# whcorkran/mamba-TTS-project

Measured on AMD Instinct MI355X. Metric: audio tokens/sec (teacher-forced fwd+bwd) per GPU; decode_step p50 latency, higher is better.
Workload: dtype bf16; 1 GPU; C2: MambaTTSDecoder 12L d_model=1024 fwd+bwd+clip+Adam, B=8/GPU T_audio=2048 T_text=128; model=MambaTTSDecoder-12L-d1024, global_batch=8, seq_len=2048, parallelism=dp1

## Files before the change

### include/mtts.h

```cpp
#ifndef MTTS_H
#define MTTS_H

#include <stdint.h>

#ifdef __cplusplus
extern "C" {
#endif

#define MTTS_ABI_VERSION 15

enum { MTTS_F32 = 0, MTTS_BF16 = 1 };
enum {
  MTTS_OK = 0,
  MTTS_EINVAL = -22,
  MTTS_EUNSUPPORTED = -95,
  MTTS_ELAUNCH = -5
};

int mtts_abi_version(void);
const char* mtts_last_error(void);

enum {
  MTTS_OVR_AUTO = -1,
  MTTS_OVR_SCAN_PATH = 0,
// ... 255 lines not shown
int mtts_embed_table_grad(const int64_t* ids, int64_t n, const void* g, int dtype, int64_t g_rs, int d, int vocab,
                          float* out, void* workspace, void* stream);

typedef struct {
  int M, N, K, act;
  int64_t ldx, ldw, ldy;
  const void* x;
  const void* W;
  const void* bias;
  void* y;
  int conv_dim;
  float* conv_state;
  const float* conv_w;
  const float* conv_b;
  void* u;
  int64_t ldu;
  const float* ln_w;
  const float* ln_b;
  float ln_eps;
  const void* gamma;
  const void* beta;
  int64_t ld_gb;
  const void* res;
  int64_t ld_res;
  int kgroups;
  float* splitk_slab;
  int* splitk_count;
  int w_packed;
  int x_packed;
  void* y_packed;
  void* u_packed;
} MttsRowsArgs;

int mtts_gemm_rows(const MttsRowsArgs* a, void* stream);

typedef struct {
  int64_t rows;
  int vocab;
  int dtype;
  int64_t ld;
  const void* logits;
  const int64_t* targets;
  int ignore_index;
  float* loss;
  float* lse;
  float* workspace;
} MttsCrossEntropyArgs;

int64_t mtts_cross_entropy_workspace(int64_t rows);
int mtts_cross_entropy_fwd(const MttsCrossEntropyArgs* a, void* stream);
int mtts_cross_entropy_bwd(const MttsCrossEntropyArgs* a, const float* grad_loss, void* dlogits, int64_t ld_dlogits,
                           void* stream);

int64_t mtts_pack_rows_bytes(int N, int K);
int mtts_pack_rows_weight(const void* W, int64_t ldw, int N, int K, void* out, void* stream);


#define MTTS_GEMM_NT 0
#define MTTS_GEMM_TN 1
#define MTTS_GEMM_EPI_BIAS 1
#define MTTS_GEMM_EPI_GELU 2
#define MTTS_GEMM_EPI_DGELU 4
typedef struct {
  int m, n, k;
  int layout;
  int splits;
  int epilogue;
  int out_dtype;
  int bias_dtype;
  int64_t lda, ldb, ldc, ld_aux;
  const void* a;
  const void* b;
  void* c;
  const void* bias;
  void* aux;
  void* workspace;
  float beta;
} MttsGemmArgs;

int64_t mtts_gemm_workspace(const MttsGemmArgs* a);
int mtts_gemm(const MttsGemmArgs* a, void* stream);

int mtts_gemm_grouped(const MttsGemmArgs* probs, int n, void* stream);

#define MTTS_CONVGEMM_NN 2
#define MTTS_CONVGEMM_BIAS 1
#define MTTS_CONVGEMM_RELU 2
#define MTTS_CONVGEMM_DRELU 4
typedef struct {
  const void* ptr;
  int64_t seg_rows, seg_stride, row_stride;
  int32_t halo_c, halo_p;
} MttsRowMap;
typedef struct {
  int layout;
  int m, n, k;
  MttsRowMap a, b, c, aux;
  const float* bias;
  int epilogue;
  float beta;
  int splits;
  void* workspace;
  float* colsum_a;
} MttsConvGemmArgs;
int64_t mtts_convgemm_workspace(const MttsConvGemmArgs* a);
int mtts_convgemm(const MttsConvGemmArgs* a, void* stream);

#define MTTS_SKINNY_N 0
#define MTTS_SKINNY_SMALL_K 1
#define MTTS_SKINNY_TN 2
typedef struct {
  int mode;
  int m, n, k;
  int c_dtype;
  float beta;
  int64_t lda, ldb, ldc;
  const void* a;
  const void* b;
  void* c;
  void* workspace;
  int trans_c;
  int reserved_;
} MttsSkinnyArgs;

int64_t mtts_gemm_skinny_workspace(const MttsSkinnyArgs* a);
int mtts_gemm_skinny(const MttsSkinnyArgs* a, void* stream);

typedef struct {
  int64_t n;
  int dtype;
  float p;
  uint64_t seed;
  const void* x;
  void* y;
  const void* pre;
  int group;
  int x_rep;
  int x_inner;
  int reserved_;
  const int64_t* seed_in;
  int64_t* seed_out;
} MttsDropoutArgs;

int mtts_dropout(const MttsDropoutArgs* a, void* stream);

typedef struct {
  int rows, vocab;
  int dtype;
  int top_k;
  int64_t ld;
  const void* logits;
  const float* bias;
  int64_t bias_ld;
  float temperature;
  float top_p;
  const int64_t* seed;
  int* step;
  int advance;
  int step0;
  int* pos;
  int64_t* tokens;
  int64_t tok_stride;
  int64_t* history;
  int64_t hist_ld;
  int hist_cols;
  int eos_id;
// ... 14 lines not shown
```

### mamba-tts-project_amd/mtts/_lib.py

```python
from __future__ import annotations

import contextlib
import ctypes as C
import os

import torch

_HERE = os.path.dirname(os.path.abspath(__file__))
LIB_PATH = os.environ.get("MTTS_LIB", os.path.join(_HERE, "libmtts.so"))
ABI_VERSION = 15

F32, BF16 = 0, 1
i32, i64, f32, vp = C.c_int, C.c_int64, C.c_float, C.c_void_p


class ScanFwdArgs(C.Structure):
    _fields_ = [("batch", i32), ("dim", i32), ("seqlen", i32), ("dstate", i32),
                ("dtype_io", i32), ("dtype_bc", i32), ("delta_softplus", i32), ("ckpt_chunk", i32),
                ("a_is_log", i32), ("reserved_", i32), ("u_bs", i64), ("u_ls", i64), ("delta_bs", i64), ("delta_ls", i64),
                ("z_bs", i64), ("z_ls", i64), ("out_bs", i64), ("out_ls", i64),
                ("B_bs", i64), ("B_ls", i64), ("C_bs", i64), ("C_ls", i64),
                ("u", vp), ("delta", vp), ("A", vp), ("Bm", vp), ("Cm", vp), ("D", vp), ("z", vp),
                ("delta_bias", vp), ("h0", vp), ("out", vp), ("last_state", vp), ("ckpt", vp),
                ("workspace", vp), ("seqlens", vp)]
# ... 72 lines not shown
class RowMap(C.Structure):
    _fields_ = [("ptr", vp), ("seg_rows", i64), ("seg_stride", i64), ("row_stride", i64), ("halo_c", i32),
                ("halo_p", i32)]


class ConvGemmArgs(C.Structure):
    _fields_ = [("layout", i32), ("m", i32), ("n", i32), ("k", i32), ("a", RowMap), ("b", RowMap), ("c", RowMap),
                ("aux", RowMap), ("bias", vp), ("epilogue", i32), ("beta", f32), ("splits", i32),
                ("workspace", vp), ("colsum_a", vp)]


class SkinnyArgs(C.Structure):
    _fields_ = [("mode", i32), ("m", i32), ("n", i32), ("k", i32), ("c_dtype", i32), ("beta", f32),
                ("lda", i64), ("ldb", i64), ("ldc", i64), ("a", vp), ("b", vp), ("c", vp), ("workspace", vp),
                ("trans_c", i32), ("reserved_", i32)]


class LNArgs(C.Structure):
    _fields_ = [("rows", i32), ("cols", i32), ("dtype", i32), ("rows_per_group", i32), ("eps", f32),
                ("x_rs", i64), ("res_rs", i64), ("xsum_rs", i64), ("y_rs", i64), ("gb_rs", i64),
                ("x", vp), ("res", vp), ("x_sum", vp), ("w", vp), ("b", vp), ("gamma", vp), ("beta", vp),
                ("gb_dtype", i32), ("y", vp), ("mean", vp), ("rstd", vp)]


class LNBwdArgs(C.Structure):
    _fields_ = [("f", LNArgs), ("dy", vp), ("dy_rs", i64), ("dx_acc", vp), ("dxacc_rs", i64),
                ("dx", vp), ("dx_rs", i64), ("dw", vp), ("db", vp), ("dgamma", vp), ("dbeta", vp),
                ("workspace", vp), ("dx_colsum", vp), ("dgb_rs", i64)]


class AttnFwdArgs(C.Structure):
    _fields_ = [("batch", i32), ("heads", i32), ("head_dim", i32), ("q_len", i32), ("kv_len", i32),
                ("dtype", i32), ("scale", f32),
                ("q_bs", i64), ("q_ls", i64), ("k_bs", i64), ("k_ls", i64), ("v_bs", i64), ("v_ls", i64),
                ("o_bs", i64), ("o_ls", i64), ("mask_bs", i64),
                ("q", vp), ("k", vp), ("v", vp), ("key_padding_mask", vp), ("out", vp), ("lse", vp),
                ("out_packed", vp), ("kv_hs", i64)]


class AttnQProjArgs(C.Structure):
    _fields_ = [("f", AttnFwdArgs), ("x", vp), ("x_rs", i64), ("wq", vp), ("bq", vp), ("ln_w", vp), ("ln_b", vp),
                ("eps", f32), ("d_model", i32)]


class AttnBwdArgs(C.Structure):
    _fields_ = [("f", AttnFwdArgs), ("dout", vp), ("do_bs", i64), ("do_ls", i64),
                ("dq", vp), ("dq_bs", i64), ("dq_ls", i64), ("dk", vp), ("dk_bs", i64), ("dk_ls", i64),
                ("dv", vp), ("dv_bs", i64), ("dv_ls", i64), ("workspace", vp)]


class CastDesc(C.Structure):
    _fields_ = [("src", vp), ("dst", vp), ("dstT", vp), ("rows", i32), ("cols", i32), ("tile0", i64)]


class AdamTensor(C.Structure):
    _fields_ = [("p", vp), ("g", vp), ("m", vp), ("v", vp), ("n", i64), ("chunk0", i64)]


_SIGS = {
    "mtts_abi_version": ([], i32),
    "mtts_last_error": ([], C.c_char_p),
    "mtts_set_override": ([i32, i32], i32),
    "mtts_get_override": ([i32], i32),
    "mtts_selective_scan_fwd_workspace": ([i32, i32, i32, i32], i64),
    "mtts_selective_scan_fwd": ([C.POINTER(ScanFwdArgs), vp], i32),
    "mtts_selective_scan_bwd_workspace": ([i32, i32, i32, i32], i64),
    "mtts_selective_scan_bwd": ([C.POINTER(ScanBwdArgs), vp], i32),
    "mtts_causal_conv1d_fwd": ([C.POINTER(ConvFwdArgs), vp], i32),
    "mtts_causal_conv1d_bwd_workspace": ([i32, i32, i32, i32], i64),
    "mtts_causal_conv1d_bwd": ([C.POINTER(ConvBwdArgs), vp], i32),
    "mtts_causal_conv1d_update": ([C.POINTER(ConvUpdateArgs), vp], i32),
    "mtts_selective_state_update": ([C.POINTER(StateUpdateArgs), vp], i32),
    "mtts_layernorm_fwd": ([C.POINTER(LNArgs), vp], i32),
    "mtts_gemm_rows": ([C.POINTER(RowsArgs), vp], i32),
    "mtts_pack_rows_bytes": ([i32, i32], i64),
    "mtts_cross_entropy_workspace": ([i64], i64),
    "mtts_cross_entropy_fwd": ([C.POINTER(CrossEntropyArgs), vp], i32),
    "mtts_cross_entropy_bwd": ([C.POINTER(CrossEntropyArgs), vp, vp, i64, vp], i32),
    "mtts_layernorm_rows_packed": ([C.POINTER(LNArgs), vp, vp], i32),
    "mtts_pack_rows_weight": ([vp, i64, i32, i32, vp, vp], i32),
    "mtts_gemm_workspace": ([C.POINTER(GemmArgs)], i64),
    "mtts_gemm": ([C.POINTER(GemmArgs), vp], i32),
    "mtts_gemm_grouped": ([C.POINTER(GemmArgs), i32, vp], i32),
    "mtts_convgemm": ([C.POINTER(ConvGemmArgs), vp], i32),
    "mtts_convgemm_workspace": ([C.POINTER(ConvGemmArgs)], i64),
    "mtts_gemm_skinny": ([C.POINTER(SkinnyArgs), vp], i32),
    "mtts_gemm_skinny_workspace": ([C.POINTER(SkinnyArgs)], i64),
    "mtts_layernorm_bwd_workspace": ([i32, i32, i32], i64),
    "mtts_layernorm_bwd": ([C.POINTER(LNBwdArgs), vp], i32),
    "mtts_colsum_workspace": ([i32, i32, i32], i64),
    "mtts_colsum": ([vp, i32, i32, i32, i64, i32, vp, i64, vp, vp], i32),
    "mtts_attention_fwd": ([C.POINTER(AttnFwdArgs), vp], i32),
    "mtts_attention_decode_qproj": ([C.POINTER(AttnQProjArgs), vp], i32),
    "mtts_attention_bwd_workspace": ([i32, i32, i32, i32, i32, i32], i64),
    "mtts_attention_bwd": ([C.POINTER(AttnBwdArgs), vp], i32),
    "mtts_adam_chunks": ([i64], i64),
    "mtts_adam_workspace": ([i64], i64),
    "mtts_clip_adam": ([vp, i32, i64, vp, f32, f32, f32, f32, f32, f32, vp, vp, vp], i32),
    "mtts_embed_sum": ([vp, i64, vp, vp, vp, vp, vp, i32, i32, i32, i32, vp, i32, i64, vp, vp], i32),
    "mtts_embed_sum_at": ([vp, i64, vp, vp, vp, vp, vp, i32, i32, i32, i32, vp, i32, i64, vp, i64, i32, vp], i32),
    "mtts_embed_table_grad_workspace": ([i64, i32, i32], i64),
    "mtts_embed_table_grad": ([vp, i64, vp, i32, i64, i32, i32, vp, vp, vp], i32),
    "mtts_cast_tiles": ([i32, i32], i64),
    "mtts_cast_bf16_multi": ([vp, i32, i64, vp], i32),
    "mtts_length_regulate_lengths": ([vp, i64, i32, i32, vp, vp], i32),
    "mtts_length_regulate_fwd": ([vp, i32, i32, i32, i32, i64, i64, vp, i64, i32, vp, i64, i64, vp], i32),
    "mtts_length_regulate_bwd": ([vp, i32, i32, i32, i32, i64, i64, vp, i64, i32, vp, i64, i64, vp], i32),
    "mtts_dropout": ([C.POINTER(DropoutArgs), vp], i32),
    "mtts_sample_tokens": ([C.POINTER(SampleArgs), vp], i32),
}

_lib = None


def lib():
    global _lib
    if _lib is None:
        if not os.path.exists(LIB_PATH):
            raise RuntimeError(f"libmtts.so not found at {LIB_PATH}; run __graft_entry__.build() "
                               "(make -C mamba-tts-project_amd/mtts/csrc)")
        L = C.CDLL(LIB_PATH)
        if not hasattr(L, "mtts_embed_sum_at"):
            raise RuntimeError(f"{LIB_PATH} is stale: it was built before mtts_embed_sum_at (ragged prompts) was "
                               "added; rebuild it with __graft_entry__.build() "
                               "(make -C mamba-tts-project_amd/mtts/csrc)")
        for name, (argt, rest) in _SIGS.items():
            fn = getattr(L, name)
            fn.argtypes = argt
            fn.restype = rest
        v = L.mtts_abi_version()
        if v != ABI_VERSION:
            raise RuntimeError(f"libmtts ABI {v} != expected {ABI_VERSION}")
        _lib = L
    return _lib


def exported_symbols():
    return list(_SIGS)


def call(name, args):
    L = lib()
    stream = torch.cuda.current_stream().cuda_stream
    rc = getattr(L, name)(C.byref(args), C.c_void_p(stream))
    if rc != 0:
        raise RuntimeError(f"{name} failed ({rc}): {L.mtts_last_error().decode()}")


def call_raw(name, *args):
    L = lib()
    rc = getattr(L, name)(*args, C.c_void_p(torch.cuda.current_stream().cuda_stream))
    if rc != 0:
        raise RuntimeError(f"{name} failed ({rc}): {L.mtts_last_error().decode()}")


OVERRIDES = {"scan_path": 0, "scan_p": 1, "scan_segs": 2, "scan_bwd_segs": 3, "gemm_narrow": 4,
             "attn_chunks": 5, "attn_bwd": 6, "attn_generic": 7, "conv_untiled": 8, "gemm_tile": 9,
             "attn_dq_dma": 10}
SCAN_C1, SCAN_W2, SCAN_NARROW = 1, 2, 3
ATTN_BWD_FUSED, ATTN_BWD_SPLIT = 1, 2


@contextlib.contextmanager
def override(**paths):
    L = lib()
    old = {}
    try:
        for k, v in paths.items():
            old[k] = L.mtts_set_override(OVERRIDES[k], -1 if v is None else int(v))
        yield
    finally:
        for k, v in old.items():
            L.mtts_set_override(OVERRIDES[k], v)


def dtype_code(t: torch.Tensor) -> int:
    if t.dtype == torch.float32:
        return F32
    if t.dtype == torch.bfloat16:
        return BF16
    raise TypeError(f"unsupported dtype {t.dtype} (libmtts takes float32 / bfloat16)")


def ptr(t):
    return None if t is None else t.data_ptr()
```

### mamba-tts-project_amd/mtts/csrc/gemm.hip

```cpp
#include "common.h"

#include <type_traits>

namespace mtts {
namespace {

typedef short s16x8 __attribute__((ext_vector_type(8)));
typedef short s16x4 __attribute__((ext_vector_type(4)));
typedef __bf16 bf16x8 __attribute__((ext_vector_type(8)));
typedef float f32x4 __attribute__((ext_vector_type(4)));
typedef __attribute__((address_space(3))) s16x4 lds_s16x4;
typedef __attribute__((address_space(3))) s16x8 lds_s16x8;

constexpr int kThreads = 512;
constexpr int kTile = 256;
constexpr int kBK = 64;
constexpr int kRegion = 16384;
constexpr int kBuf = 4 * kRegion;
constexpr int kLds = 2 * kBuf;

enum { R_A0 = 0, R_A1 = 1, R_B0 = 2, R_B1 = 3 };

struct GemmParams {
  const bf16_t* a;
  const bf16_t* b;
  void* c;
  const void* bias;
  void* aux;
  int64_t lda, ldb, ldc, ld_aux;
  int64_t split_stride;
  int m, n, k;
  int tiles_m, tiles_n, splits;
  int group;
  int epi;
  int bias_bf16;
  int wide_out;
  float beta;
};

__device__ __forceinline__ int a_map(int rr, int s) { return (rr >> 6) * 128 + s * 64 + (rr & 63); }
__device__ __forceinline__ int b_map(int rr, int s) { return (rr >> 5) * 64 + s * 32 + (rr & 31); }
template <bool IS_A>
__device__ __forceinline__ int rmap(int rr, int s) { return IS_A ? a_map(rr, s) : b_map(rr, s); }

__device__ __forceinline__ void glds16(const void* base, uint32_t voff, uint32_t lds_base) {
#if defined(__HIP_DEVICE_COMPILE__)
  asm volatile("s_mov_b32 m0, %2\n\ts_nop 0\n\tglobal_load_lds_dwordx4 %0, %1" ::"v"(voff), "s"(base), "s"(lds_base)
               : "memory", "m0");
#endif
}
template <int N>
__device__ __forceinline__ void wait_vm() {
#if defined(__HIP_DEVICE_COMPILE__)
  static_assert(N >= 0 && N < 64, "vmcnt range");
  __builtin_amdgcn_s_waitcnt((N & 15) | (7 << 4) | (15 << 8) | ((N >> 4) << 14));
#endif
}
__device__ __forceinline__ void barrier() {
#if defined(__HIP_DEVICE_COMPILE__)
  __builtin_amdgcn_s_waitcnt(0xC07F);
#ifndef MTTS_GEMM_DIAG_NOBAR
  __builtin_amdgcn_s_barrier();
#endif
  asm volatile("" ::: "memory");
#endif
}

__device__ __forceinline__ f32x4 mfma(s16x8 a, s16x8 b, f32x4 c) {
  return __builtin_amdgcn_mfma_f32_16x16x32_bf16(__builtin_bit_cast(bf16x8, a), __builtin_bit_cast(bf16x8, b), c, 0,
                                                 0, 0);
}

__device__ __forceinline__ float gelu_tail_s(float a) {
  float s = -1.7774024116e-08f;
  s = fmaf(s, a, 5.6194854933e-07f);
  s = fmaf(s, a, -7.6223902631e-06f);
  s = fmaf(s, a, 5.5893204013e-05f);
  s = fmaf(s, a, -2.0454518331e-04f);
  s = fmaf(s, a, -1.6655060660e-04f);
  s = fmaf(s, a, 7.1668288485e-03f);
  s = fmaf(s, a, -5.2604280745e-02f);
  s = fmaf(s, a, 2.6218665810e-01f);
  s = fmaf(s, a, -1.1511125488e+00f);
  s = fmaf(s, a, -9.9999981719e-01f);
// ... 680 lines not shown
  if (wr == 1) sbar();

  const char* lbase = lds;
  s16x8 af[2][4], b0f[2][2], b1f[2][2];
#define PP_MFMA(BF, MO, NO)                                                                   \
  __builtin_amdgcn_sched_barrier(0);                                                        \
  __builtin_amdgcn_s_waitcnt(0xC07F);                                                        \
  __builtin_amdgcn_sched_barrier(0);                                                        \
  __builtin_amdgcn_s_setprio(1);                                                            \
  _Pragma("unroll") for (int ks_ = 0; ks_ < 2; ++ks_)                                        \
  _Pragma("unroll") for (int mb_ = 0; mb_ < 4; ++mb_)                                        \
  _Pragma("unroll") for (int nb_ = 0; nb_ < 2; ++nb_)                                        \
      acc[(MO) + mb_][(NO) + nb_] = mfma(BF[ks_][nb_], af[ks_][mb_], acc[(MO) + mb_][(NO) + nb_]); \
  __builtin_amdgcn_s_setprio(0);                                                            \
  __builtin_amdgcn_sched_barrier(0);                                                        \
  sbar();
  for (int g = 0; g < G; ++g) {
    const bool steady = g > 0 && g + 2 < G;
    const bool n1 = g + 1 < G, n2 = g + 2 < G;
    const char* bufp = lbase + (g & 1) * kBuf;
#pragma unroll
    for (int ks = 0; ks < 2; ++ks) {
#pragma unroll
      for (int nb = 0; nb < 2; ++nb) b0f[ks][nb] = frag<BKM>(bufp + R_B0 * kRegion, wc * 32 + nb * 16, ks, lane);
#pragma unroll
      for (int mb = 0; mb < 4; ++mb) af[ks][mb] = frag<AK>(bufp + R_A0 * kRegion, wr * 64 + mb * 16, ks, lane);
    }
    if (n1) stage(g + 1, R_A1);
    if (steady) wait_ops<6>();
    else wait_ops_rt<6>(g == 0 ? (n1 ? 8 : 2) : (n1 ? 6 : 0));
    sbar();
    PP_MFMA(b0f, 0, 0)
#pragma unroll
    for (int ks = 0; ks < 2; ++ks)
#pragma unroll
      for (int nb = 0; nb < 2; ++nb) b1f[ks][nb] = frag<BKM>(bufp + R_B1 * kRegion, wc * 32 + nb * 16, ks, lane);
    if (n1) stage(g + 1, R_B1);
    if (steady) wait_ops<10>();
    else wait_ops_rt<10>(g == 0 ? (n1 ? 8 : 0) : (n1 ? 10 : 2));
    sbar();
    PP_MFMA(b1f, 0, 2)
#pragma unroll
    for (int ks = 0; ks < 2; ++ks)
#pragma unroll
      for (int mb = 0; mb < 4; ++mb) af[ks][mb] = frag<AK>(bufp + R_A1 * kRegion, wr * 64 + mb * 16, ks, lane);
    if (n2) stage(g + 2, R_A0);
    sbar();
    PP_MFMA(b1f, 4, 2)
    if (n2) stage(g + 2, R_B0);
    if (steady) wait_ops<8>();
    else if (n1) wait_ops_rt<8>((n2 ? 8 : 4));
    sbar();
    PP_MFMA(b0f, 4, 0)
  }
#undef PP_MFMA
  if (wr == 0) sbar();
  store_tile_buf<EPI, OUT_F32>(p, acc, bias, cur.m0, cur.n0, wr, wc, lane, cur.split);
}

template <bool AK, bool BKM, int EPI, bool OUT_F32>
__global__ __launch_bounds__(kThreads, 1) void gemm_pp_kernel(GemmParams p) {
  gemm_pp_body<AK, BKM, EPI, OUT_F32>(p, xcd_work_id());
}

constexpr int kGroupMax = 24;
struct GroupParams {
  GemmParams p[kGroupMax];
  int tile_end[kGroupMax];
  int n;
};

template <bool AK, bool BKM, int EPI, bool OUT_F32>
__global__ __launch_bounds__(kThreads, 1) void gemm_pp_grouped_kernel(const GroupParams G) {
  const int wid = xcd_work_id();
  int i = 0, t0 = 0;
#pragma unroll
  for (int j = 0; j + 1 < kGroupMax; ++j)
    if (j + 1 < G.n && wid >= G.tile_end[j]) { i = j + 1; t0 = G.tile_end[j]; }
  GemmParams q = G.p[0];
#pragma unroll
  for (int j = 1; j < kGroupMax; ++j)
    if (i == j) q = G.p[j];
  gemm_pp_body<AK, BKM, EPI, OUT_F32>(q, wid - t0);
}

constexpr int kW4Threads = 256;
constexpr int kW4BK = 32;
constexpr int kW4Stages = 4;
constexpr int kW4Stage = 32768;

__device__ __forceinline__ int w4_slot(int r, int c) { return 4 * r + (c ^ (-(r >> 2) & 3)); }

template <int EPI>
__global__ __launch_bounds__(kW4Threads, 1) void gemm_w4_kernel(GemmParams p) {
  __shared__ __attribute__((aligned(16))) char lds[kW4Stages * kW4Stage];
  const int tid = threadIdx.x, lane = tid & 63, wave = __builtin_amdgcn_readfirstlane(tid >> 6);
  const int wr = wave >> 1, wc = wave & 1;
  const int nk = p.k / kW4BK;
  const WorkItem it = work_item(p, xcd_work_id());
  const uint32_t lds0 = (uint32_t)(uintptr_t)(__attribute__((address_space(3))) char*)lds;

  uint32_t oa[4], ob[4];
  {
    const int r = lane >> 2;
    const int c = (lane & 3) ^ (-(r >> 2) & 3);
#pragma unroll
    for (int i = 0; i < 4; ++i) {
      int row = it.m0 + (4 * wave + i) * 16 + r;
      row = row < p.m ? row : p.m - 1;
      oa[i] = (uint32_t)((int64_t)row * p.lda * 2) + c * 16;
      int col = it.n0 + (4 * wave + i) * 16 + r;
      col = col < p.n ? col : p.n - 1;
      ob[i] = (uint32_t)((int64_t)col * p.ldb * 2) + c * 16;
    }
  }
  const char* abase = (const char*)p.a;
  const char* bbase = (const char*)p.b;
  auto stage1 = [&](int g, int slot, int j) {
    const uint32_t st = lds0 + slot * kW4Stage + wave * 4096;
    if (j < 4) glds16(abase + g * (kW4BK * 2), oa[j & 3], st + (j & 3) * 1024);
    else glds16(bbase + g * (kW4BK * 2), ob[j & 3], st + 16384 + (j & 3) * 1024);
  };
  const char* fra = lds + wr * 8192 + w4_slot(lane & 15, lane >> 4) * 16;
  const char* frb = fra - wr * 8192 + 16384 + wc * 8192;
  auto fa = [&](int g, int mb) -> s16x8 { return *(const lds_s16x8*)(fra + (g & 3) * kW4Stage + mb * 1024); };
  auto fb = [&](int g, int nb) -> s16x8 { return *(const lds_s16x8*)(frb + (g & 3) * kW4Stage + nb * 1024); };

  f32x4 acc[2][8][4];
#pragma unroll
  for (int h = 0; h < 2; ++h)
#pragma unroll
    for (int i = 0; i < 8; ++i)
#pragma unroll
      for (int j = 0; j < 4; ++j) acc[h][i][j] = f32x4{0.f, 0.f, 0.f, 0.f};

#pragma unroll
  for (int g = 0; g < kW4Stages; ++g)
#pragma unroll
    for (int j = 0; j < 8; ++j) stage1(g < nk ? g : nk - 1, g, j);
  wait_ops<24>();
  sbar();
  s16x8 fA[8], fB[2][8];
#pragma unroll
  for (int j = 0; j < 8; ++j) {
    fA[j] = fa(0, j);
    fB[0][j] = fb(0, j);
  }

  auto step = [&](int g, auto cur_c) {
    constexpr int CUR = decltype(cur_c)::value;
    wait_ops<16>();
    barrier();
    const int gs = g + 4 < nk ? g + 4 : nk - 1;
#pragma unroll
    for (int j = 0; j < 8; ++j) {
      __builtin_amdgcn_sched_barrier(0);
      stage1(gs, (g + 4) & 3, j);
#pragma unroll
      for (int nb = 0; nb < 8; ++nb)
        acc[nb >> 2][j][nb & 3] = mfma(fB[CUR][nb], fA[j], acc[nb >> 2][j][nb & 3]);
      fA[j] = fa(g + 1, j);
      fB[1 - CUR][j] = fb(g + 1, j);
    }
    __builtin_amdgcn_sched_barrier(0);
  };
  for (int g = 0; g < nk; g += 2) {
// ... 91 lines not shown
  MTTS_CHECK((epi & (MTTS_GEMM_EPI_GELU | MTTS_GEMM_EPI_DGELU)) != (MTTS_GEMM_EPI_GELU | MTTS_GEMM_EPI_DGELU),
             "gemm: GELU and DGELU are exclusive");
  MTTS_CHECK(nt || (epi == 0 && f32out), "gemm: TN (weight gradient) runs fp32 out, no epilogue");
  MTTS_CHECK(splits == 1 || a->workspace, "gemm: split-K needs the workspace (mtts_gemm_workspace bytes)");

  GemmParams p{};
  p.a = (const bf16_t*)a->a; p.b = (const bf16_t*)a->b;
  p.bias = a->bias; p.aux = a->aux; p.bias_bf16 = a->bias_dtype == 1;
  p.lda = a->lda; p.ldb = a->ldb; p.ld_aux = a->ld_aux;
  p.m = M; p.n = N; p.k = K / splits;
  p.tiles_m = (M + kTile - 1) / kTile; p.tiles_n = (N + kTile - 1) / kTile;
  p.splits = splits; p.epi = epi;
  p.group = std::min(p.tiles_m, 4);
  if (splits > 1) {
    p.c = a->workspace; p.ldc = N; p.split_stride = (int64_t)M * N; p.beta = 0.f;
  } else {
    p.c = a->c; p.ldc = a->ldc; p.split_stride = 0; p.beta = a->beta;
  }
  p.wide_out = !f32out && a->ldc % 8 == 0 && (!(epi & (MTTS_GEMM_EPI_GELU | MTTS_GEMM_EPI_DGELU)) || a->ld_aux % 8 == 0) &&
               (!a->aux || (uintptr_t)a->aux % 16 == 0) && override_of(MTTS_OVR_GEMM_NARROW) != 1;
  const int nwg = p.tiles_m * p.tiles_n * splits;
  hipStream_t st = (hipStream_t)stream;
  if (!nt) {
    launch<false, false, 0, true>(p, nwg, st);
  } else if (f32out) {
    launch<true, true, 0, true>(p, nwg, st);
  } else {
    switch (epi) {
      case 0: launch<true, true, 0, false>(p, nwg, st); break;
      case MTTS_GEMM_EPI_BIAS: launch<true, true, MTTS_GEMM_EPI_BIAS, false>(p, nwg, st); break;
      case MTTS_GEMM_EPI_GELU: launch<true, true, MTTS_GEMM_EPI_GELU, false>(p, nwg, st); break;
      case MTTS_GEMM_EPI_BIAS | MTTS_GEMM_EPI_GELU:
        launch<true, true, MTTS_GEMM_EPI_BIAS | MTTS_GEMM_EPI_GELU, false>(p, nwg, st); break;
      case MTTS_GEMM_EPI_DGELU: launch<true, true, MTTS_GEMM_EPI_DGELU, false>(p, nwg, st); break;
      default: MTTS_CHECK(false, "gemm: unsupported epilogue combination %d", epi);
    }
  }
  MTTS_LAUNCH_CHECK("gemm");
  if (splits > 1) {
    const int64_t total = (int64_t)M * (N / 4);
    const int blocks = (int)std::min<int64_t>((total + 255) / 256, 2048);
    hipLaunchKernelGGL(split_reduce_kernel, dim3(blocks), dim3(256), 0, st, (const float*)a->workspace,
                       (int64_t)M * N, splits, M, N, (int64_t)N, (float*)a->c, a->ldc, a->beta);
    MTTS_LAUNCH_CHECK("gemm split reduce");
  }
  return MTTS_OK;
}

extern "C" int mtts_gemm_grouped(const MttsGemmArgs* probs, int n, void* stream) {
  using namespace mtts;
  MTTS_CHECK(probs && n >= 1 && n <= kGroupMax, "gemm_grouped: 1 <= n <= %d problems", kGroupMax);
  GroupParams G{};
  int tiles = 0;
  for (int i = 0; i < n; ++i) {
    const MttsGemmArgs* a = probs + i;
    MTTS_CHECK(a->a && a->b && a->c, "gemm_grouped[%d]: null pointer", i);
    const int M = a->m, N = a->n, K = a->k;
    MTTS_CHECK(a->layout == MTTS_GEMM_TN && a->out_dtype == 0 && a->epilogue == 0 && a->splits <= 1,
               "gemm_grouped[%d]: TN, fp32 out, no epilogue, no split-K only", i);
    MTTS_CHECK(M > 0 && N > 0 && K > 0 && K % kBK == 0, "gemm_grouped[%d]: m=%d n=%d k=%d (k %% 64 == 0)", i, M, N, K);
    MTTS_CHECK(N % 8 == 0 && M % 8 == 0, "gemm_grouped[%d]: m, n must be multiples of 8", i);
    MTTS_CHECK(((uintptr_t)a->a | (uintptr_t)a->b) % 16 == 0 && a->lda % 8 == 0 && a->ldb % 8 == 0 &&
               a->lda >= M && a->ldb >= N, "gemm_grouped[%d]: A / B alignment or leading dimension", i);
    MTTS_CHECK(a->ldc % 4 == 0 && (uintptr_t)a->c % 16 == 0 && a->ldc >= N, "gemm_grouped[%d]: C alignment / ldc", i);
    MTTS_CHECK(a->beta == 0.f || a->beta == 1.f, "gemm_grouped[%d]: beta must be 0 or 1", i);
    MTTS_CHECK((int64_t)(kBK - 1) * a->lda + M < (1ll << 31) && (int64_t)(kBK - 1) * a->ldb + N < (1ll << 31) &&
               (int64_t)M * a->ldc * 4 < (1ll << 31), "gemm_grouped[%d]: operand / C span exceeds the 32-bit offsets", i);
    GemmParams& p = G.p[i];
    p.a = (const bf16_t*)a->a; p.b = (const bf16_t*)a->b; p.c = a->c;
    p.lda = a->lda; p.ldb = a->ldb; p.ldc = a->ldc;
    p.m = M; p.n = N; p.k = K;
    p.tiles_m = (M + kTile - 1) / kTile; p.tiles_n = (N + kTile - 1) / kTile;
    p.splits = 1; p.split_stride = 0; p.beta = a->beta;
    p.group = std::min(p.tiles_m, 4);
    tiles += p.tiles_m * p.tiles_n;
    G.tile_end[i] = tiles;
  }
  G.n = n;
  hipLaunchKernelGGL((gemm_pp_grouped_kernel<false, false, 0, true>), dim3(tiles), dim3(kThreads), 0,
                     (hipStream_t)stream, G);
  MTTS_LAUNCH_CHECK("gemm_grouped");
  return MTTS_OK;
}
```

### mamba-tts-project_amd/mtts/wgrad.py

```python
from __future__ import annotations

import contextlib
import ctypes as C

import torch

from . import _lib as L
from . import gemm as G

GROUP_TILES = 192
MAX_PROBLEMS = 24
MIN_GROUP_TILES = 128
SIDE_STREAM = False

_depth = 0


class _Job:
    __slots__ = ("dy", "x", "param", "rows")

    def __init__(self, dy, x, param, rows):
        self.dy, self.x, self.param, self.rows = dy, x, param, rows

    def tiles(self):
        m, n = self.dy.shape[1], self.x.shape[1]
        return -(-m // G.TILE) * -(-n // G.TILE)


class _Engine:
    def __init__(self):
        self.jobs = []
        self.tiles = 0
        self.callback_queued = False
        self.done = set()
        self.covered = {}
        self.listeners = []
        self.side = {}
        self.used_side = None

    def reset_pass(self):
        self.callback_queued = False
        self.done = set()
        self.covered = {}
        self.used_side = None


_E = _Engine()


def active() -> bool:
    return _depth > 0


@contextlib.contextmanager
def deferred(enable: bool = True):
    global _depth
    if not enable:
        yield
        return
    _depth += 1
    try:
        yield
    finally:
        _depth -= 1
        if _depth == 0 and (_E.jobs or _E.used_side is not None):
            _end_of_backward()


def owns(p) -> bool:
    if id(p) in _E.done:
        return False
    return id(p) in _E.covered or any(j.param is p for j in _E.jobs)


def add_listener(fn):
    _E.listeners.append(fn)


def remove_listener(fn):
    if fn in _E.listeners:
        _E.listeners.remove(fn)


def _eligible(dy, x, param, narrow=False):
    return (active() and param is not None and param.requires_grad and param.dtype == torch.float32
            and param.dim() == 2 and (narrow or (dy.shape[1] >= 256 and x.shape[1] >= 256)) and G.tn_ok(dy, x))


def _end_of_backward():
    flush()
    if _E.used_side is not None:
        main, side = _E.used_side
        main.wait_stream(side)
    for key, (p, _, _) in list(_E.covered.items()):
        if key not in _E.done:
            _announce(p)
    _E.reset_pass()


def _announce(p):
    _E.done.add(id(p))
    for fn in _E.listeners:
        fn(p)


def _cover(p, rows):
    r0, r1 = rows if rows is not None else (0, p.shape[0])
    _, ivs, overlap = _E.covered.get(id(p), (p, [], False))
    overlap = overlap or any(a < r1 and r0 < b for a, b in ivs)
    ivs = ivs + [(r0, r1)]
    _E.covered[id(p)] = (p, ivs, overlap)
    if overlap:
        return False
    return sum(b - a for a, b in ivs) >= p.shape[0]


def _side_stream(dev):
    i = dev.index if dev.index is not None else torch.cuda.current_device()
    st = _E.side.get(i)
    if st is None:
        st = _E.side[i] = torch.cuda.Stream(device=i)
    return st


def submit(jobs, narrow=False) -> bool:
    if not jobs or not all(_eligible(dy, x, p, narrow) for dy, x, p, _ in jobs):
        return False
    param = jobs[0][2]
    for dy, x, p, rows in jobs:
        r0, r1 = rows if rows is not None else (0, p.shape[0])
        if p is not param or p.shape[1] != x.shape[1] or r1 - r0 != dy.shape[1]:
            return False
    if id(param) in _E.done and _E.listeners:
        raise RuntimeError("wgrad: a parameter's weight gradient was submitted after its gradient was announced "
                           "complete to a listener (a weight used again later in the backward under GradAllReduce); "
                           "run this backward outside mtts.wgrad.deferred()")
    if any(j.param is param for j in _E.jobs):
        flush()
    if not _E.callback_queued:
        torch.autograd.Variable._execution_engine.queue_callback(_end_of_backward)
        _E.callback_queued = True
    for dy, x, p, rows in jobs:
        j = _Job(dy, x, p, rows)
        _E.jobs.append(j)
        _E.tiles += j.tiles()
    if _E.tiles >= GROUP_TILES or len(_E.jobs) >= MAX_PROBLEMS - 2:
        flush()
    return True


def flush():
    jobs, _E.jobs, _E.tiles = _E.jobs, [], 0
    if not jobs:
        return
    if not (SIDE_STREAM and _E.callback_queued):
        _flush(jobs)
        return
    main = torch.cuda.current_stream()
    side = _side_stream(jobs[0].dy.device)
    side.wait_stream(main)
    _E.used_side = (main, side)
    for j in jobs:
        j.dy.record_stream(side)
        j.x.record_stream(side)
    with torch.cuda.stream(side):
        _flush(jobs, side)


def _flush(jobs, side=None):
    dest = {}
    for j in jobs:
        p = j.param
        if id(p) in dest:
            continue
        if p.grad is not None:
            dest[id(p)] = (p.grad, 1.0, False)
            continue
        cover = sum((j2.rows[1] - j2.rows[0]) if j2.rows else p.shape[0] for j2 in jobs if j2.param is p)
        view = getattr(p, "_mtts_grad_view", None)
        full = cover >= p.shape[0]
        if view is not None:
            if not full:
                view.zero_()
            g = view
        else:
            g = torch.empty(p.shape, device=p.device, dtype=torch.float32) if full else \
                torch.zeros(p.shape, device=p.device, dtype=torch.float32)
        if side is not None:
            g.record_stream(side)
        dest[id(p)] = (g, 0.0 if full else 1.0, True)
    probs, fixups = [], []
    for j in jobs:
        g, beta, _ = dest[id(j.param)]
        out = g if j.rows is None else g[j.rows[0]:j.rows[1]]
        if not _addressable(out):
            tmp = torch.empty(out.shape, device=out.device, dtype=torch.float32)
            if side is not None:
                tmp.record_stream(side)
            fixups.append((out, tmp, beta))
            out, beta = tmp, 0.0
        probs.append((j.dy, j.x, out, beta))
    probs.sort(key=lambda t: -t[0].shape[0])
    if sum(-(-dy.shape[1] // G.TILE) * -(-x.shape[1] // G.TILE) for dy, x, _, _ in probs) < MIN_GROUP_TILES:
        for dy, x, out, beta in probs:
            G.mm_tn(dy, x, out=out, beta=beta)
    else:
        for s in range(0, len(probs), MAX_PROBLEMS):
            _launch(probs[s:s + MAX_PROBLEMS])
    for out, tmp, beta in fixups:
        if beta:
            out.add_(tmp)
        else:
            out.copy_(tmp)
    for j in jobs:
        g, _, fresh = dest[id(j.param)]
        if fresh and j.param.grad is None:
            j.param.grad = g
    complete = {}
    for j in jobs:
        if _cover(j.param, j.rows) and id(j.param) not in _E.done:
            complete[id(j.param)] = j.param
    for p in complete.values():
        _announce(p)


def _addressable(out):
    return out.stride(1) == 1 and out.stride(0) % 4 == 0 and out.data_ptr() % 16 == 0


def _launch(probs):
    arr = (L.GemmArgs * len(probs))()
    for a, (dy, x, out, beta) in zip(arr, probs):
        k, m = dy.shape
        n = x.shape[1]
        if not _addressable(out) or tuple(out.shape) != (m, n):
            raise RuntimeError("wgrad: gradient destination not 16-byte addressable")
        a.m, a.n, a.k, a.layout, a.splits, a.out_dtype = m, n, k, G.TN, 1, 0
        a.lda, a.ldb, a.ldc = dy.stride(0), x.stride(0), out.stride(0)
        a.a, a.b, a.c = dy.data_ptr(), x.data_ptr(), out.data_ptr()
        a.beta = beta
    lib = L.lib()
    rc = lib.mtts_gemm_grouped(arr, len(probs), C.c_void_p(torch.cuda.current_stream().cuda_stream))
    if rc != 0:
        raise RuntimeError(f"mtts_gemm_grouped failed ({rc}): {lib.mtts_last_error().decode()}")
```

Measured before the change: 522,800 tokens/s.

## Batch weight-gradient GEMMs across layers to fill full CU rounds

Adds a grouped TN GEMM kernel that takes up to 64 problems and maps work ids to XCDs round by round. The weight-gradient engine now holds jobs from several layers, using a makespan model to pick how many layer groups to batch before flushing. The aim is fewer partially filled waves and launch tails on the CUs. In exchange, activations stay alive longer (capped by a byte budget), gradient production is delayed, and a plain O(n) cover computation replaces the quadratic one.

```diff
diff --git a/include/mtts.h b/include/mtts.h
--- a/include/mtts.h
+++ b/include/mtts.h
@@ -361,6 +361,8 @@
 int mtts_gemm(const MttsGemmArgs* a, void* stream);
 
 int mtts_gemm_grouped(const MttsGemmArgs* probs, int n, void* stream);
+
+int mtts_gemm_grouped_rounds(const MttsGemmArgs* probs, int n, void* stream);
 
 #define MTTS_CONVGEMM_NN 2
 #define MTTS_CONVGEMM_BIAS 1
diff --git a/mamba-tts-project_amd/mtts/_lib.py b/mamba-tts-project_amd/mtts/_lib.py
--- a/mamba-tts-project_amd/mtts/_lib.py
+++ b/mamba-tts-project_amd/mtts/_lib.py
@@ -178,6 +178,7 @@
     "mtts_gemm_workspace": ([C.POINTER(GemmArgs)], i64),
     "mtts_gemm": ([C.POINTER(GemmArgs), vp], i32),
     "mtts_gemm_grouped": ([C.POINTER(GemmArgs), i32, vp], i32),
+    "mtts_gemm_grouped_rounds": ([C.POINTER(GemmArgs), i32, vp], i32),
     "mtts_convgemm": ([C.POINTER(ConvGemmArgs), vp], i32),
     "mtts_convgemm_workspace": ([C.POINTER(ConvGemmArgs)], i64),
     "mtts_gemm_skinny": ([C.POINTER(SkinnyArgs), vp], i32),
@@ -216,10 +217,12 @@
             raise RuntimeError(f"libmtts.so not found at {LIB_PATH}; run __graft_entry__.build() "
                                "(make -C mamba-tts-project_amd/mtts/csrc)")
         L = C.CDLL(LIB_PATH)
-        if not hasattr(L, "mtts_embed_sum_at"):
-            raise RuntimeError(f"{LIB_PATH} is stale: it was built before mtts_embed_sum_at (ragged prompts) was "
-                               "added; rebuild it with __graft_entry__.build() "
-                               "(make -C mamba-tts-project_amd/mtts/csrc)")
+        for sym, what in (("mtts_embed_sum_at", "ragged prompts"),
+                          ("mtts_gemm_grouped_rounds", "round-filling weight gradients")):
+            if not hasattr(L, sym):
+                raise RuntimeError(f"{LIB_PATH} is stale: it was built before {sym} ({what}) was "
+                                   "added; rebuild it with __graft_entry__.build() "
+                                   "(make -C mamba-tts-project_amd/mtts/csrc)")
         for name, (argt, rest) in _SIGS.items():
             fn = getattr(L, name)
             fn.argtypes = argt
diff --git a/mamba-tts-project_amd/mtts/csrc/gemm.hip b/mamba-tts-project_amd/mtts/csrc/gemm.hip
--- a/mamba-tts-project_amd/mtts/csrc/gemm.hip
+++ b/mamba-tts-project_amd/mtts/csrc/gemm.hip
@@ -1,5 +1,7 @@
 #include "common.h"
 
+#include <algorithm>
+#include <cstddef>
 #include <type_traits>
 
 namespace mtts {
@@ -846,6 +848,58 @@
   for (int j = 1; j < kGroupMax; ++j)
     if (i == j) q = G.p[j];
   gemm_pp_body<AK, BKM, EPI, OUT_F32>(q, wid - t0);
+}
+
+constexpr int kRoundsMax = 64;
+struct RoundProb {
+  const bf16_t* a;
+  const bf16_t* b;
+  void* c;
+  int lda, ldb, ldc;
+  int m, n, k;
+  float beta;
+  int pad_;
+};
+struct RoundParams {
+  RoundProb p[kRoundsMax];
+  int tile_end[kRoundsMax];
+  int n;
+  int round;
+};
+static_assert(sizeof(RoundProb) == 56 && offsetof(RoundParams, p) == 0 && sizeof(RoundParams) <= 4096,
+              "round-filling problem table must fit the kernel arguments");
+static_assert(offsetof(RoundProb, lda) == 24 && offsetof(RoundProb, ldc) == 32 && offsetof(RoundProb, n) == 40 &&
+              offsetof(RoundProb, beta) == 48, "gemm_pp_rounds_kernel reads RoundProb as qwords");
+
+__device__ __forceinline__ int round_work_id(int round) {
+  const int bid = blockIdx.x;
+  const int b = bid % round, r0 = bid - b;
+  const int nwg = min(round, (int)gridDim.x - r0);
+  const int q8 = nwg / 8, r8 = nwg % 8, xcd = b % 8;
+  return r0 + (xcd < r8 ? xcd * (q8 + 1) : r8 * (q8 + 1) + (xcd - r8) * q8) + b / 8;
+}
+
+__global__ __launch_bounds__(kThreads, 1) void gemm_pp_rounds_kernel(const RoundParams G) {
+  const int wid = round_work_id(G.round);
+  int i = 0, t0 = 0;
+#pragma unroll
+  for (int j = 0; j + 1 < kRoundsMax; ++j)
+    if (j + 1 < G.n && wid >= G.tile_end[j]) { i = j + 1; t0 = G.tile_end[j]; }
+  GemmParams q{};
+#if defined(__HIP_DEVICE_COMPILE__)
+  typedef const __attribute__((address_space(4))) uint64_t* KArg;
+  const KArg e = (KArg)__builtin_amdgcn_kernarg_segment_ptr() +
+                 __builtin_amdgcn_readfirstlane(i) * (int)(sizeof(RoundProb) / 8);
+  const uint64_t ld_ab = e[3], ldc_m = e[4], n_k = e[5];
+  q.a = (const bf16_t*)e[0]; q.b = (const bf16_t*)e[1]; q.c = (void*)e[2];
+  q.lda = (int)(uint32_t)ld_ab; q.ldb = (int)(ld_ab >> 32); q.ldc = (int)(uint32_t)ldc_m;
+  q.m = (int)(ldc_m >> 32); q.n = (int)(uint32_t)n_k; q.k = (int)(n_k >> 32);
+  q.beta = __uint_as_float((uint32_t)e[6]);
+#endif
+  q.tiles_m = (q.m + kTile - 1) / kTile; q.tiles_n = (q.n + kTile - 1) / kTile;
+  q.splits = 1;
+  q.group = min(q.tiles_m, 4);
+  gemm_pp_body<false, false, 0, true>(q, wid - t0);
 }
 
 constexpr int kW4Threads = 256;
@@ -1103,3 +1157,47 @@
   MTTS_LAUNCH_CHECK("gemm_grouped");
   return MTTS_OK;
 }
+
+extern "C" int mtts_gemm_grouped_rounds(const MttsGemmArgs* probs, int n, void* stream) {
+  using namespace mtts;
+  MTTS_CHECK(probs && n >= 1 && n <= kRoundsMax, "gemm_grouped_rounds: 1 <= n <= %d problems", kRoundsMax);
+  RoundParams G{};
+  int64_t tiles = 0;
+  for (int i = 0; i < n; ++i) {
+    const MttsGemmArgs* a = probs + i;
+    MTTS_CHECK(a->a && a->b && a->c, "gemm_grouped_rounds[%d]: null pointer", i);
+    const int M = a->m, N = a->n, K = a->k;
+    MTTS_CHECK(a->layout == MTTS_GEMM_TN && a->out_dtype == 0 && a->epilogue == 0 && a->splits <= 1,
+               "gemm_grouped_rounds[%d]: TN, fp32 out, no epilogue, no split-K only", i);
+    MTTS_CHECK(M > 0 && N > 0 && K > 0 && K % kBK == 0, "gemm_grouped_rounds[%d]: m=%d n=%d k=%d (k %% 64 == 0)", i, M, N,
+               K);
+    MTTS_CHECK(N % 8 == 0 && M % 8 == 0, "gemm_grouped_rounds[%d]: m, n must be multiples of 8", i);
+    MTTS_CHECK(((uintptr_t)a->a | (uintptr_t)a->b) % 16 == 0 && a->lda % 8 == 0 && a->ldb % 8 == 0 &&
+               a->lda >= M && a->ldb >= N, "gemm_grouped_rounds[%d]: A / B alignment or leading dimension", i);
+    MTTS_CHECK(a->ldc % 4 == 0 && (uintptr_t)a->c % 16 == 0 && a->ldc >= N, "gemm_grouped_rounds[%d]: C alignment / ldc",
+               i);
+    MTTS_CHECK(a->beta == 0.f || a->beta == 1.f, "gemm_grouped_rounds[%d]: beta must be 0 or 1", i);
+    MTTS_CHECK((int64_t)(kBK - 1) * a->lda + M < (1ll << 31) && (int64_t)(kBK - 1) * a->ldb + N < (1ll << 31) &&
+               (int64_t)M * a->ldc * 4 < (1ll << 31),
+               "gemm_grouped_rounds[%d]: operand / C span exceeds the 32-bit offsets", i);
+    RoundProb& p = G.p[i];
+    p.a = (const bf16_t*)a->a; p.b = (const bf16_t*)a->b; p.c = a->c;
+    p.lda = (int)a->lda; p.ldb = (int)a->ldb; p.ldc = (int)a->ldc;
+    p.m = M; p.n = N; p.k = K;
+    p.beta = a->beta;
+    tiles += (int64_t)((M + kTile - 1) / kTile) * ((N + kTile - 1) / kTile);
+    MTTS_CHECK(tiles < (1ll << 31), "gemm_grouped_rounds[%d]: more than 2^31 output tiles", i);
+    G.tile_end[i] = (int)tiles;
+  }
+  G.n = n;
+  int dev = 0, cus = 0;
+  if (hipGetDevice(&dev) != hipSuccess ||
+      hipDeviceGetAttribute(&cus, hipDeviceAttributeMultiprocessorCount, dev) != hipSuccess) {
+    (void)hipGetLastError();
+    cus = 0;
+  }
+  G.round = std::max(8, cus / 8 * 8);
+  hipLaunchKernelGGL(gemm_pp_rounds_kernel, dim3((unsigned)tiles), dim3(kThreads), 0, (hipStream_t)stream, G);
+  MTTS_LAUNCH_CHECK("gemm_grouped_rounds");
+  return MTTS_OK;
+}
diff --git a/mamba-tts-project_amd/mtts/wgrad.py b/mamba-tts-project_amd/mtts/wgrad.py
--- a/mamba-tts-project_amd/mtts/wgrad.py
+++ b/mamba-tts-project_amd/mtts/wgrad.py
@@ -2,6 +2,7 @@
 
 import contextlib
 import ctypes as C
+import heapq
 
 import torch
 
@@ -9,7 +10,13 @@
 from . import gemm as G
 
 GROUP_TILES = 192
-MAX_PROBLEMS = 24
+MAX_PROBLEMS = 64
+LAYER_PROBLEMS = 24
+FILL_ROUNDS = True
+FILL = 0.95
+HOLD_BYTES = 6 << 30
+_LAYER_TILES = GROUP_TILES
+_BK = 64
 MIN_GROUP_TILES = 128
 SIDE_STREAM = False
 
@@ -25,12 +32,97 @@
     def tiles(self):
         m, n = self.dy.shape[1], self.x.shape[1]
         return -(-m // G.TILE) * -(-n // G.TILE)
+
+    def nbytes(self):
+        return self.dy.numel() * self.dy.element_size() + self.x.numel() * self.x.element_size()
+
+
+def makespan(work, cus):
+    by_k = {}
+    for t, k in work:
+        if t > 0 and k > 0:
+            by_k[k] = by_k.get(k, 0) + t
+    loads = [0] * cus
+    for k in sorted(by_k, reverse=True):
+        t = by_k[k]
+        if loads[-1] - loads[0] > k:
+            heapq.heapify(loads)
+            top = max(loads)
+            while t and top - loads[0] > k:
+                new = loads[0] + k
+                heapq.heapreplace(loads, new)
+                top = max(top, new)
+                t -= 1
+            loads.sort()
+        q, r = divmod(t, cus)
+        if q:
+            loads = [v + q * k for v in loads]
+        if r:
+            loads[:r] = [v + k for v in loads[:r]]
+            loads.sort()
+    return loads[-1]
+
+
+def utilisation(work, cus):
+    total = sum(t * k for t, k in work if t > 0 and k > 0)
+    return total / (cus * makespan(work, cus)) if total else 0.0
+
+
+def plan_groups(work, nbytes, cus):
+    n = 1
+    while n * len(work) <= MAX_PROBLEMS - 2 and n * nbytes <= HOLD_BYTES:
+        if utilisation(work * n, cus) >= FILL:
+            return n
+        n += 1
+    return 1
+
+
+class RoundQueue:
+
+    def __init__(self):
+        self.clear()
+
+    def clear(self):
+        self.work = []
+        self.held = 0
+        self.tiles = 0
+        self.jobs = 0
+        self.groups = 0
+        self.plan = 1
+
+    def add(self, tiles, ktiles, nbytes):
+        self.work.append((tiles, ktiles))
+        self.held += nbytes
+        self.tiles += tiles
+        self.jobs += 1
+
+    def full(self, cus):
+        if len(self.work) >= MAX_PROBLEMS - 2:
+            return True
+        if self.tiles < GROUP_TILES and self.jobs < LAYER_PROBLEMS - 2:
+            return False
+        self.tiles = self.jobs = 0
+        self.groups += 1
+        if self.groups == 1:
+            self.plan = plan_groups(self.work, self.held, cus)
+        return self.groups >= self.plan or self.held >= HOLD_BYTES
+
+
+_cus = {}
+
+
+def cu_count(dev):
+    i = dev.index if dev.index is not None else torch.cuda.current_device()
+    if i not in _cus:
+        _cus[i] = torch.cuda.get_device_properties(i).multi_processor_count
+    return _cus[i]
 
 
 class _Engine:
     def __init__(self):
         self.jobs = []
         self.tiles = 0
+        self.queue = RoundQueue()
         self.callback_queued = False
         self.done = set()
         self.covered = {}
@@ -144,13 +236,18 @@
         j = _Job(dy, x, p, rows)
         _E.jobs.append(j)
         _E.tiles += j.tiles()
-    if _E.tiles >= GROUP_TILES or len(_E.jobs) >= MAX_PROBLEMS - 2:
+        _E.queue.add(j.tiles(), dy.shape[0] // _BK, j.nbytes())
+    if not FILL_ROUNDS or _E.listeners or GROUP_TILES < _LAYER_TILES:
+        if _E.tiles >= GROUP_TILES or len(_E.jobs) >= LAYER_PROBLEMS - 2:
+            flush()
+    elif _E.queue.full(cu_count(dy.device)):
         flush()
     return True
 
 
 def flush():
     jobs, _E.jobs, _E.tiles = _E.jobs, [], 0
+    _E.queue.clear()
     if not jobs:
         return
     if not (SIDE_STREAM and _E.callback_queued):
@@ -168,7 +265,9 @@
 
 
 def _flush(jobs, side=None):
-    dest = {}
+    dest, covered = {}, {}
+    for j in jobs:
+        covered[id(j.param)] = covered.get(id(j.param), 0) + ((j.rows[1] - j.rows[0]) if j.rows else j.param.shape[0])
     for j in jobs:
         p = j.param
         if id(p) in dest:
@@ -176,7 +275,7 @@
         if p.grad is not None:
             dest[id(p)] = (p.grad, 1.0, False)
             continue
-        cover = sum((j2.rows[1] - j2.rows[0]) if j2.rows else p.shape[0] for j2 in jobs if j2.param is p)
+        cover = covered[id(p)]
         view = getattr(p, "_mtts_grad_view", None)
         full = cover >= p.shape[0]
         if view is not None:
@@ -240,6 +339,6 @@
         a.a, a.b, a.c = dy.data_ptr(), x.data_ptr(), out.data_ptr()
         a.beta = beta
     lib = L.lib()
-    rc = lib.mtts_gemm_grouped(arr, len(probs), C.c_void_p(torch.cuda.current_stream().cuda_stream))
+    rc = lib.mtts_gemm_grouped_rounds(arr, len(probs), C.c_void_p(torch.cuda.current_stream().cuda_stream))
     if rc != 0:
-        raise RuntimeError(f"mtts_gemm_grouped failed ({rc}): {lib.mtts_last_error().decode()}")
+        raise RuntimeError(f"mtts_gemm_grouped_rounds failed ({rc}): {lib.mtts_last_error().decode()}")
```

Measured after the change: 529,000 tokens/s (median of 6 runs). 1.2% higher.
